# kezakool/flair-for-aigle

Measured on AMD Instinct MI355X. Metric: 512x512x5 tiles/sec (train fwd+bwd+AdamW), U-Net ResNet-34, 19 classes, higher is better.
Workload: dtype bf16; 1 GPU; synthetic 512x512x5 tiles, 19-class U-Net (ResNet-34 encoder), batch 32 per GPU, train step (BASELINE.json configs[1]); global_batch=32, tile=512, parallelism=dp1

## Files before the change

flair-for-aigle_amd/csrc/norm_pool.hip:

```cpp
#include "ffa_common.h"

#define FFA_EW_THREADS 256
#define FFA_MAX_PARTIALS 1024
#ifndef FFA_EW_UNROLL
#define FFA_EW_UNROLL 4
#endif

static inline int ew_grid(long long items) {
  long long g = (items + FFA_EW_THREADS - 1) / FFA_EW_THREADS;
  if (g > 256 * 8) g = 256 * 8;
  if (g < 1) g = 1;
  return (int)g;
}

static inline int ew_grid_c(long long nvec, int C) {
  int a = C / 8, b = FFA_EW_THREADS;
  while (b) {
    const int r = a % b;
    a = b;
    b = r;
  }
  const int m = (C / 8) / a;
  const int g = ew_grid((nvec + FFA_EW_UNROLL - 1) / FFA_EW_UNROLL) / m * m;
  return g < m ? m : g;
// ... 867 lines not shown
    red[t][e] = a[e];
    red[t][8 + e] = b[e];
  }
  __syncthreads();
  const int PL = FFA_COOP_THREADS / CG;
  for (int idx = t; idx < 2 * C; idx += FFA_COOP_THREADS) {
    const int which = idx / C, c = idx % C;
    const int g = c / 8, e = (c % 8) + which * 8;
    float s = 0.f;
    for (int q = 0; q < PL; ++q) s += red[q * CG + g][e];
    ws[((long long)blockIdx.x * 2 + which) * C + c] = s;
  }
  const unsigned nb = gridDim.x;
  bool ok = ffa_grid_barrier(sync + 0, nb, sync + 3);
  float* tot = ws + (long long)FFA_MAX_PARTIALS * 2 * C;
  for (int v = blockIdx.x; v < 2 * C; v += nb) {
    double s = 0.0;
    for (unsigned p = t; p < nb; p += FFA_COOP_THREADS) s += (double)ws[(long long)p * 2 * C + v];
#pragma unroll
    for (int o = 32; o > 0; o >>= 1) s += __shfl_xor(s, o, 64);
    if ((t & 63) == 0) dred[t >> 6] = s;
    __syncthreads();
    if (t == 0) {
      double r = 0.0;
      for (int wv = 0; wv < FFA_COOP_THREADS / 64; ++wv) r += dred[wv];
      tot[v] = (float)r;
    }
    __syncthreads();
  }
  ok = ffa_grid_barrier(sync + 1, nb, sync + 3) && ok;
  float kg[8], kx[8], k0[8];
#pragma unroll
  for (int e = 0; e < 8; ++e) {
    const float s = __hip_atomic_load(tot + c0 + e, __ATOMIC_RELAXED, __HIP_MEMORY_SCOPE_AGENT);
    const float q = __hip_atomic_load(tot + C + c0 + e, __ATOMIC_RELAXED, __HIP_MEMORY_SCOPE_AGENT);
    kg[e] = (gamma ? gamma[c0 + e] : 1.f) * rs[e];
    kx[e] = -kg[e] * rs[e] * q * inv_count;
    k0[e] = -kg[e] * s * inv_count - kx[e] * mu[e];
    if (blockIdx.x == 0 && t < CG) {
      dbeta[c0 + e] = s;
      dgamma[c0 + e] = q;
    }
  }
#pragma unroll
  for (int k = 0; k < ITEMS; ++k) {
    const long long i = tid_g + (long long)k * nthreads;
    if (i < nvec) {
      float xv[8], gv[8], o[8];
      ffa_unpack8_bf16(xr[k], xv);
      ffa_unpack8_bf16(gr[k], gv);
#pragma unroll
      for (int e = 0; e < 8; ++e) o[e] = kg[e] * gv[e] + kx[e] * xv[e] + k0[e];
      ffa_store8<ffa_bf16>(dx + i * 8, o);
      if (dres) *reinterpret_cast<ffa_u32x4*>(dres + i * 8) = gr[k];
    }
  }
  __syncthreads();
  if (t == 0) {
    __threadfence();
    if (atomicAdd(sync + 2, 1u) == nb - 1) {
      sync[0] = 0u;
      sync[1] = 0u;
      sync[2] = 0u;
      __threadfence();
    }
  }
  (void)ok;
}

extern "C" int ffa_bn_bwd_fused(int dtype, const void* x, const void* dy, const void* y, const float* gamma,
                                const float* beta, const float* mean, const float* rstd, void* dx, void* dres,
                                float* dgamma, float* dbeta, long long npix, int C, int relu, void* workspace,
                                long long workspace_bytes, unsigned* sync, hipStream_t stream) {
  FFA_REQUIRE(x && dy && dx && mean && rstd && dgamma && dbeta && workspace && sync, "bn_bwd_fused: null pointer");
  FFA_REQUIRE(relu >= 0 && relu <= 2 && (relu != 1 || y), "bn_bwd_fused: bad relu mode");
  static int cus = 0;
  if (cus == 0) {
    int dev = 0;
    hipDeviceProp_t prop;
    if (hipGetDevice(&dev) != hipSuccess || hipGetDeviceProperties(&prop, dev) != hipSuccess) return FFA_ERR_UNSUPPORTED;
    cus = prop.multiProcessorCount;
  }
  const int CG = C / 8;
  if (dtype != FFA_BF16 || C % 8 != 0 || CG < 1 || FFA_COOP_THREADS % CG != 0 || cus < 8 || cus > FFA_MAX_PARTIALS) {
    ffa_set_error("bn_bwd_fused: unsupported dtype / channel count %d", C);
    return FFA_ERR_UNSUPPORTED;
  }
  if (workspace_bytes < ffa_bn_workspace_bytes(C)) {
    ffa_set_error("bn_bwd_fused: workspace too small");
    return FFA_ERR_WORKSPACE;
  }
  const long long nvec = npix * CG;
  const long long nthreads = (long long)cus * FFA_COOP_THREADS;
  const long long items = (nvec + nthreads - 1) / nthreads;
  if (items > 16) {
    ffa_set_error("bn_bwd_fused: %lld vectors per thread exceed the register budget", items);
    return FFA_ERR_UNSUPPORTED;
  }
  const float inv_count = (float)(1.0 / (double)npix);
#define FFA_COOP_LAUNCH(N_)                                                                                      \
  hipLaunchKernelGGL(bn_bwd_coop_kernel<N_>, dim3(cus), dim3(FFA_COOP_THREADS), 0, stream, (const ffa_bf16*)x,   \
                     (const ffa_bf16*)dy, (const ffa_bf16*)y, gamma, beta, mean, rstd, (ffa_bf16*)dx,            \
                     (ffa_bf16*)dres, dgamma, dbeta, (float*)workspace, sync, nvec, C, relu, inv_count)
  if (items <= 4) FFA_COOP_LAUNCH(4);
  else FFA_COOP_LAUNCH(16);
#undef FFA_COOP_LAUNCH
  return ffa_check_launch("bn_bwd_fused");
}

extern "C" int ffa_bn_bwd_partials(int dtype, const void* x, const void* dy, const float* partials, long long nparts,
                                   const float* gamma, const float* beta, const float* mean, const float* rstd,
                                   void* dx, float* dgamma, float* dbeta, long long npix, int C, void* workspace,
                                   long long workspace_bytes, hipStream_t stream) {
  FFA_REQUIRE(x && dy && partials && dx && mean && rstd && dgamma && dbeta && workspace, "bn_bwd_partials: null pointer");
  FFA_REQUIRE(C % 8 == 0 && C >= 8 && C <= 8 * FFA_EW_THREADS && nparts > 0, "bn_bwd_partials: bad arguments");
  if (workspace_bytes < ffa_bn_workspace_bytes(C)) {
    ffa_set_error("bn_bwd_partials: workspace too small");
    return FFA_ERR_WORKSPACE;
  }
  float* ws = static_cast<float*>(workspace);
  float* coef = ws + (long long)FFA_MAX_PARTIALS * 2 * C;
  const float* src = partials;
  int n = (int)nparts;
  if (nparts > FFA_MAX_PARTIALS) {
    const int R = 64;
    hipLaunchKernelGGL(partials_fold_kernel, dim3(ffa_cdiv(C, 8), R), dim3(FFA_FIN_THREADS), 0, stream, partials, nparts,
                       C, R, ws);
    src = ws;
    n = R;
  }
  const long long nvec = npix * (C / 8);
  const float inv_count = (float)(1.0 / (double)npix);
  hipLaunchKernelGGL(bn_bwd_finalize_kernel, dim3(ffa_cdiv(C, 8)), dim3(FFA_FIN_THREADS), 0, stream, src, n, C, gamma, beta,
                     mean, rstd, inv_count, dgamma, dbeta, coef, 1);
  if (dtype == FFA_BF16)
    hipLaunchKernelGGL(bn_bwd_apply_kernel<ffa_bf16>, dim3(ew_grid_c(nvec, C)), dim3(FFA_EW_THREADS), 0, stream,
                       (const ffa_bf16*)x, (const ffa_bf16*)dy, (const ffa_bf16*)nullptr, coef, (ffa_bf16*)dx,
                       (ffa_bf16*)nullptr, nvec, C, 2);
  else
    hipLaunchKernelGGL(bn_bwd_apply_kernel<float>, dim3(ew_grid_c(nvec, C)), dim3(FFA_EW_THREADS), 0, stream, (const float*)x,
                       (const float*)dy, (const float*)nullptr, coef, (float*)dx, (float*)nullptr, nvec, C, 2);
  return ffa_check_launch("bn_bwd_partials");
}


template <typename T>
__global__ void __launch_bounds__(FFA_EW_THREADS)
maxpool_fwd_kernel(const T* __restrict__ x, T* __restrict__ y, uint8_t* __restrict__ idx, int B, int H, int W, int C,
                   int Ho, int Wo) {
  const unsigned CG = C / 8;
  const int oy = blockIdx.x % Ho;
  const long long b = blockIdx.x / Ho;
  const long long row = (long long)blockIdx.x * Wo * CG;
  for (unsigned j = threadIdx.x; j < (unsigned)Wo * CG; j += FFA_EW_THREADS) {
    const int ox = (int)(j / CG), g = (int)(j % CG);
    const long long i = row + j;
    float best[8];
    int bi[8];
#pragma unroll
    for (int e = 0; e < 8; ++e) {
      best[e] = -INFINITY;
      bi[e] = 0;
    }
    bool first = true;
#pragma unroll
    for (int r = 0; r < 3; ++r) {
      const int iy = oy * 2 - 1 + r;
      if (iy < 0 || iy >= H) continue;
#pragma unroll
      for (int s = 0; s < 3; ++s) {
        const int ix = ox * 2 - 1 + s;
        if (ix < 0 || ix >= W) continue;
        float v[8];
        ffa_load8<T>(x + ((b * H + iy) * W + ix) * C + g * 8, v);
#pragma unroll
        for (int e = 0; e < 8; ++e) {
          if (first || v[e] > best[e] || v[e] != v[e]) {
            best[e] = v[e];
            bi[e] = r * 3 + s;
          }
        }
        first = false;
      }
    }
    ffa_store8<T>(y + i * 8, best);
    uint32_t lo = bi[0] | (bi[1] << 8) | (bi[2] << 16) | (bi[3] << 24);
    uint32_t hi = bi[4] | (bi[5] << 8) | (bi[6] << 16) | (bi[7] << 24);
    *reinterpret_cast<uint2*>(idx + i * 8) = make_uint2(lo, hi);
  }
}

template <typename T>
__global__ void __launch_bounds__(FFA_EW_THREADS)
maxpool_bwd_kernel(const T* __restrict__ dy, const uint8_t* __restrict__ idx, const T* __restrict__ add,
                   T* __restrict__ dx, int B, int H, int W, int C, int Ho, int Wo) {
  const unsigned CG = C / 8;
  const int iy = blockIdx.x % H;
  const long long b = blockIdx.x / H;
  const long long row = (long long)blockIdx.x * W * CG;
  for (unsigned j = threadIdx.x; j < (unsigned)W * CG; j += FFA_EW_THREADS) {
    const int ix = (int)(j / CG), g = (int)(j % CG);
    const long long i = row + j;
    const int ny = (iy & 1) ? 2 : 1, nx = (ix & 1) ? 2 : 1;
    const int oy_c[2] = {(iy & 1) ? (iy + 1) >> 1 : iy >> 1, (iy - 1) >> 1};
    const int r_c[2] = {(iy & 1) ? 0 : 1, 2};
    const int ox_c[2] = {(ix & 1) ? (ix + 1) >> 1 : ix >> 1, (ix - 1) >> 1};
    const int s_c[2] = {(ix & 1) ? 0 : 1, 2};
    float acc[8];
#pragma unroll
    for (int e = 0; e < 8; ++e) acc[e] = 0.f;
    Raw8<T> addr, gr[4];
    uint2 kk[4];
    bool ok[4];
    if (add) addr.load(add + i * 8);
#pragma unroll
    for (int c = 0; c < 4; ++c) {
      const int cy = c >> 1, cx = c & 1;
      ok[c] = cy < ny && cx < nx && oy_c[cy] >= 0 && oy_c[cy] < Ho && ox_c[cx] >= 0 && ox_c[cx] < Wo;
      const long long o = ok[c] ? (((b * Ho + oy_c[cy]) * Wo + ox_c[cx]) * CG + g) * 8 : 0;
      kk[c] = *reinterpret_cast<const uint2*>(idx + o);
      gr[c].load(dy + o);
    }
    if (add) addr.get(acc);
#pragma unroll
    for (int c = 0; c < 4; ++c) {
      if (!ok[c]) continue;
      const int tap = r_c[c >> 1] * 3 + s_c[c & 1];
      float gv[8];
      gr[c].get(gv);
#pragma unroll
      for (int e = 0; e < 8; ++e) {
        const uint32_t word = e < 4 ? kk[c].x : kk[c].y;
        const int wq = (word >> (8 * (e & 3))) & 0xff;
        if (wq == tap) acc[e] += gv[e];
      }
    }
    ffa_store8<T>(dx + i * 8, acc);
  }
}

extern "C" int ffa_maxpool3x3s2_fwd(int dtype, const void* x, void* y, uint8_t* idx, int B, int H, int W, int C,
                                    hipStream_t stream) {
  FFA_REQUIRE(x && y && idx && C % 8 == 0, "maxpool_fwd: bad arguments");
  const int Ho = (H + 2 - 3) / 2 + 1, Wo = (W + 2 - 3) / 2 + 1;
  FFA_REQUIRE(B > 0 && (long long)B * Ho < (1LL << 31), "maxpool_fwd: too many rows");
  const int rows = B * Ho;
  if (dtype == FFA_BF16)
    hipLaunchKernelGGL(maxpool_fwd_kernel<ffa_bf16>, dim3(rows), dim3(FFA_EW_THREADS), 0, stream,
                       (const ffa_bf16*)x, (ffa_bf16*)y, idx, B, H, W, C, Ho, Wo);
  else
    hipLaunchKernelGGL(maxpool_fwd_kernel<float>, dim3(rows), dim3(FFA_EW_THREADS), 0, stream,
                       (const float*)x, (float*)y, idx, B, H, W, C, Ho, Wo);
  return ffa_check_launch("maxpool_fwd");
}

extern "C" int ffa_maxpool3x3s2_bwd(int dtype, const void* dy, const uint8_t* idx, const void* add, void* dx, int B,
                                    int H, int W, int C, hipStream_t stream) {
  FFA_REQUIRE(dy && dx && idx && C % 8 == 0, "maxpool_bwd: bad arguments");
  const int Ho = (H + 2 - 3) / 2 + 1, Wo = (W + 2 - 3) / 2 + 1;
  FFA_REQUIRE(B > 0 && (long long)B * H < (1LL << 31), "maxpool_bwd: too many rows");
  const int rows = B * H;
  if (dtype == FFA_BF16)
    hipLaunchKernelGGL(maxpool_bwd_kernel<ffa_bf16>, dim3(rows), dim3(FFA_EW_THREADS), 0, stream,
                       (const ffa_bf16*)dy, idx, (const ffa_bf16*)add, (ffa_bf16*)dx, B, H, W, C, Ho, Wo);
  else
    hipLaunchKernelGGL(maxpool_bwd_kernel<float>, dim3(rows), dim3(FFA_EW_THREADS), 0, stream,
                       (const float*)dy, idx, (const float*)add, (float*)dx, B, H, W, C, Ho, Wo);
  return ffa_check_launch("maxpool_bwd");
}

extern "C" int ffa_channel_sums(int dtype, const void* x, long long npix, int C, float* sum_out, float* sumsq_out,
                                void* workspace, long long workspace_bytes, hipStream_t stream) {
  FFA_REQUIRE(x && sum_out && sumsq_out && workspace, "channel_sums: null pointer");
  FFA_REQUIRE(C % 8 == 0 && C >= 8 && C <= 8 * FFA_EW_THREADS, "channel_sums: unsupported channel count %d", C);
  if (workspace_bytes < ffa_bn_workspace_bytes(C)) {
    ffa_set_error("channel_sums: workspace too small");
    return FFA_ERR_WORKSPACE;
  }
  const int nb = reduce_blocks(npix, C);
  float* ws = static_cast<float*>(workspace);
  if (dtype == FFA_BF16)
    hipLaunchKernelGGL((channel_reduce_kernel<ffa_bf16, StatOp>), dim3(nb), dim3(FFA_EW_THREADS), 0, stream,
                       (const ffa_bf16*)x, (const ffa_bf16*)nullptr, (const ffa_bf16*)nullptr, nullptr, nullptr, nullptr, nullptr, ws,
                       npix, C, 0, (ffa_bf16*)nullptr);
  else
    hipLaunchKernelGGL((channel_reduce_kernel<float, StatOp>), dim3(nb), dim3(FFA_EW_THREADS), 0, stream,
                       (const float*)x, (const float*)nullptr, (const float*)nullptr, nullptr, nullptr, nullptr, nullptr, ws, npix,
                       C, 0, (float*)nullptr);
  hipLaunchKernelGGL(bn_bwd_finalize_kernel, dim3(ffa_cdiv(C, 8)), dim3(FFA_FIN_THREADS), 0, stream, ws, nb, C,
                     (const float*)nullptr, (const float*)nullptr, (const float*)nullptr, (const float*)nullptr, 0.f,
                     sumsq_out, sum_out, (float*)nullptr);
  return ffa_check_launch("channel_sums");
}
```

flair-for-aigle_amd/csrc/resample_loss.hip:

```cpp
#include "ffa_common.h"

#include <stdlib.h>

#define FFA_EW_THREADS 256

static inline int ew_grid(long long items) {
  long long g = (items + FFA_EW_THREADS - 1) / FFA_EW_THREADS;
  if (g > 256 * 8) g = 256 * 8;
  if (g < 1) g = 1;
  return (int)g;
}


template <typename T>
__global__ void up2_concat_fwd_kernel(const T* __restrict__ lo, const T* __restrict__ skip, T* __restrict__ out, int B,
                                      int Hl, int Wl, int C1, int C2) {
  const int H = Hl * 2, W = Wl * 2, C = C1 + C2;
  const int CG = C / 8, CG1 = C1 / 8;
  const long long total = (long long)B * H * W * CG;
  for (long long i = blockIdx.x * (long long)blockDim.x + threadIdx.x; i < total;
       i += (long long)gridDim.x * blockDim.x) {
    const int g = (int)(i % CG);
    long long p = i / CG;
    const int x = (int)(p % W);
// ... 183 lines not shown
  else
    hipLaunchKernelGGL(bilinear_fwd_kernel<float>, dim3(ew_grid(items)), dim3(FFA_EW_THREADS), 0, stream,
                       (const float*)x, (float*)y, B, Hi, Wi, Ho, Wo, C, sy, sx);
  return ffa_check_launch("bilinear_fwd");
}

extern "C" long long ffa_bilinear_bwd_workspace_bytes(int B, int Hi, int Wi, int C) {
  (void)B; (void)Hi; (void)Wi; (void)C;
  return 0;
}

extern "C" int ffa_bilinear_bwd(int dtype, const void* dy, void* dx, int B, int Hi, int Wi, int Ho, int Wo, int C,
                                void* workspace, long long workspace_bytes, hipStream_t stream) {
  (void)workspace; (void)workspace_bytes;
  FFA_REQUIRE(dy && dx && C % 8 == 0 && B > 0 && Hi > 0 && Wi > 0 && Ho > 0 && Wo > 0, "bilinear_bwd: bad arguments");
  const float sy = (float)Hi / (float)Ho, sx = (float)Wi / (float)Wo;
  const long long items = (long long)B * Hi * Wi * (C / 8);
  if (dtype == FFA_BF16)
    hipLaunchKernelGGL(bilinear_bwd_kernel<ffa_bf16>, dim3(ew_grid(items)), dim3(FFA_EW_THREADS), 0, stream,
                       (const ffa_bf16*)dy, (ffa_bf16*)dx, B, Hi, Wi, Ho, Wo, C, sy, sx);
  else
    hipLaunchKernelGGL(bilinear_bwd_kernel<float>, dim3(ew_grid(items)), dim3(FFA_EW_THREADS), 0, stream,
                       (const float*)dy, (float*)dx, B, Hi, Wi, Ho, Wo, C, sy, sx);
  return ffa_check_launch("bilinear_bwd");
}


#define FFA_CE_BLOCKS 1024

__global__ void ce_weight_sum_kernel(const uint8_t* __restrict__ tgt, const float* __restrict__ w, int K,
                                     long long npix, float* __restrict__ parts, int vec16) {
  __shared__ float red[FFA_EW_THREADS / 64];
  __shared__ float wl[256];
  for (int i = threadIdx.x; i < 256; i += blockDim.x) wl[i] = (i < K) ? w[i] : 0.f;
  __syncthreads();
  float s = 0.f;
  const long long gid = blockIdx.x * (long long)blockDim.x + threadIdx.x;
  const long long stride = (long long)gridDim.x * blockDim.x;
  long long done = 0;
  if (vec16) {
    const long long n16 = npix / 16;
    for (long long i = gid; i < n16; i += stride) {
      const uint4 v = reinterpret_cast<const uint4*>(tgt)[i];
      const uint32_t q[4] = {v.x, v.y, v.z, v.w};
#pragma unroll
      for (int j = 0; j < 4; ++j)
#pragma unroll
        for (int b = 0; b < 4; ++b) s += wl[(q[j] >> (8 * b)) & 0xff];
    }
    done = n16 * 16;
  }
  for (long long i = done + gid; i < npix; i += stride) s += wl[tgt[i]];
  s = ffa_wave_sum(s);
  if ((threadIdx.x & 63) == 0) red[threadIdx.x >> 6] = s;
  __syncthreads();
  if (threadIdx.x == 0) {
    float tot = 0.f;
    for (int k = 0; k < FFA_EW_THREADS / 64; ++k) tot += red[k];
    parts[blockIdx.x] = tot;
  }
}

__device__ __forceinline__ double ce_sum_partials(const float* __restrict__ parts, int n) {
  double s = 0.0;
  for (int i = threadIdx.x; i < n; i += 64) s += (double)parts[i];
#pragma unroll
  for (int o = 32; o > 0; o >>= 1) s += __shfl_xor(s, o, 64);
  return s;
}

__global__ void ce_finalize_sum_kernel(const float* __restrict__ parts, int n, float* __restrict__ out) {
  const double s = ce_sum_partials(parts, n);
  if (threadIdx.x == 0) out[0] = (float)s;
}

__global__ void ce_finalize_loss_kernel(const float* __restrict__ parts, int n, const float* __restrict__ wsum,
                                        float* __restrict__ loss) {
  const double s = ce_sum_partials(parts, n);
  if (threadIdx.x == 0) loss[0] = (float)(s / (double)wsum[0]);
}

template <typename T>
__global__ void __launch_bounds__(FFA_EW_THREADS)
softmax_ce_kernel(const T* __restrict__ logits, const uint8_t* __restrict__ tgt, const float* __restrict__ w,
                  const float* __restrict__ wsum, const float* __restrict__ grad_scale, T* __restrict__ dlogits,
                  uint8_t* __restrict__ pred, float* __restrict__ parts, long long npix, int K, int Cp) {
  __shared__ float red[FFA_EW_THREADS / 64];
  float lsum = 0.f;
  float gs = 0.f;
  if (dlogits) gs = grad_scale[0] / wsum[0];
  const int nv = Cp / 8;
  for (long long i = blockIdx.x * (long long)blockDim.x + threadIdx.x; i < npix;
       i += (long long)gridDim.x * blockDim.x) {
    float z[FFA_CE_MAXK];
#pragma unroll
    for (int v = 0; v < FFA_CE_MAXK / 8; ++v) {
      if (v < nv) {
        float tmp[8];
        ffa_load8<T>(logits + i * Cp + v * 8, tmp);
#pragma unroll
        for (int e = 0; e < 8; ++e) z[v * 8 + e] = tmp[e];
      }
    }
    float m = -INFINITY;
    int am = 0;
#pragma unroll
    for (int k = 0; k < FFA_CE_MAXK; ++k) {
      if (k < K && z[k] > m) {
        m = z[k];
        am = k;
      }
    }
    const int t = tgt[i];
    const float wt = (t < K) ? w[t] : 0.f;
    float se = 0.f, dt = 0.f;
#pragma unroll
    for (int k = 0; k < FFA_CE_MAXK; ++k) {
      if (k < K) {
        const float d = z[k] - m;
        if (k == t) dt = d;
        z[k] = __expf(d);
        se += z[k];
      }
    }
    const float inv = 1.f / se;
    if (wt != 0.f) lsum += wt * (__logf(se) - dt);
    if (pred) pred[i] = (uint8_t)am;
    if (dlogits) {
      const float c = wt * gs;
#pragma unroll
      for (int v = 0; v < FFA_CE_MAXK / 8; ++v) {
        if (v < nv) {
          float o[8];
#pragma unroll
          for (int e = 0; e < 8; ++e) {
            const int k = v * 8 + e;
            o[e] = (k < K) ? c * (z[k] * inv - (k == t ? 1.f : 0.f)) : 0.f;
          }
          ffa_store8<T>(dlogits + i * Cp + v * 8, o);
        }
      }
    }
  }
  lsum = ffa_wave_sum(lsum);
  if ((threadIdx.x & 63) == 0) red[threadIdx.x >> 6] = lsum;
  __syncthreads();
  if (threadIdx.x == 0) {
    float tot = 0.f;
    for (int k = 0; k < FFA_EW_THREADS / 64; ++k) tot += red[k];
    parts[blockIdx.x] = tot;
  }
}

template <typename T, bool SUMS>
__global__ void __launch_bounds__(FFA_EW_THREADS)
softmax_ce_tiled_kernel(const T* __restrict__ logits, const uint8_t* __restrict__ tgt, const float* __restrict__ w,
                        const float* __restrict__ wsum, const float* __restrict__ grad_scale, T* __restrict__ dlogits,
                        uint8_t* __restrict__ pred, float* __restrict__ parts, float* __restrict__ parts_b,
                        long long npix, int K, int Cp) {
  constexpr int EPP = 16 / (int)sizeof(T);
  constexpr int MAXP = FFA_CE_MAXK / EPP;
  __shared__ __align__(16) unsigned char tile[FFA_EW_THREADS * (MAXP + 1) * 16];
  __shared__ float red[FFA_EW_THREADS / 64];
  const int tid = threadIdx.x;
  const int np = Cp / EPP;
  const int slots = np | 1;
  float bsum[SUMS ? EPP : 1];
#pragma unroll
  for (int k = 0; k < (SUMS ? EPP : 1); ++k) bsum[k] = 0.f;
  float lsum = 0.f;
  float gs = 0.f;
  if (dlogits) gs = grad_scale[0] / wsum[0];
  const long long ntiles = (npix + FFA_EW_THREADS - 1) / FFA_EW_THREADS;
  int loff[MAXP];
#pragma unroll
  for (int k = 0; k < MAXP; ++k) {
    const int idx = tid + FFA_EW_THREADS * k;
    loff[k] = ((idx / np) * slots + idx % np) * 16;
  }
  uint4 pre[MAXP];
  auto gload = [&](long long ti) {
    const long long base = ti * FFA_EW_THREADS;
    const long long left = npix - base;
    const int npc = (int)(left < FFA_EW_THREADS ? left : FFA_EW_THREADS) * np;
    const uint4* src = reinterpret_cast<const uint4*>(logits + base * Cp);
#pragma unroll
    for (int k = 0; k < MAXP; ++k) {
      const int idx = tid + FFA_EW_THREADS * k;
      if (k < np) pre[k] = idx < npc ? src[idx] : make_uint4(0u, 0u, 0u, 0u);
    }
  };
  long long ti = blockIdx.x;
  if (ti < ntiles) gload(ti);
  for (; ti < ntiles; ti += gridDim.x) {
#pragma unroll
    for (int k = 0; k < MAXP; ++k)
      if (k < np) *reinterpret_cast<uint4*>(tile + loff[k]) = pre[k];
    __syncthreads();
    if (ti + gridDim.x < ntiles) gload(ti + gridDim.x);
    const long long i = ti * FFA_EW_THREADS + tid;
    if (i < npix) {
      unsigned char* mine = tile + tid * slots * 16;
      float z[FFA_CE_MAXK];
#pragma unroll
      for (int v = 0; v < MAXP; ++v) {
        if (v < np) {
          const uint4 u = *reinterpret_cast<const uint4*>(mine + v * 16);
          if constexpr (sizeof(T) == 2) {
            z[v * 8 + 0] = __uint_as_float(u.x << 16);
            z[v * 8 + 1] = __uint_as_float(u.x & 0xffff0000u);
            z[v * 8 + 2] = __uint_as_float(u.y << 16);
            z[v * 8 + 3] = __uint_as_float(u.y & 0xffff0000u);
            z[v * 8 + 4] = __uint_as_float(u.z << 16);
            z[v * 8 + 5] = __uint_as_float(u.z & 0xffff0000u);
            z[v * 8 + 6] = __uint_as_float(u.w << 16);
            z[v * 8 + 7] = __uint_as_float(u.w & 0xffff0000u);
          } else {
            z[v * 4 + 0] = __uint_as_float(u.x);
            z[v * 4 + 1] = __uint_as_float(u.y);
            z[v * 4 + 2] = __uint_as_float(u.z);
            z[v * 4 + 3] = __uint_as_float(u.w);
          }
        }
      }
      float m = -INFINITY;
      int am = 0;
#pragma unroll
      for (int k = 0; k < FFA_CE_MAXK; ++k) {
        if (k < K && z[k] > m) {
          m = z[k];
          am = k;
        }
      }
      const int t = tgt[i];
      const float wt = (t < K) ? w[t] : 0.f;
      float se = 0.f, dt = 0.f;
#pragma unroll
      for (int k = 0; k < FFA_CE_MAXK; ++k) {
        if (k < K) {
          const float d = z[k] - m;
          if (k == t) dt = d;
          z[k] = __expf(d);
          se += z[k];
        }
      }
      const float inv = 1.f / se;
      if (wt != 0.f) lsum += wt * (__logf(se) - dt);
      if (pred) pred[i] = (uint8_t)am;
      if (dlogits) {
        const float c = wt * gs;
#pragma unroll
        for (int v = 0; v < MAXP; ++v) {
          if (v < np) {
            float o[EPP];
#pragma unroll
            for (int e = 0; e < EPP; ++e) {
              const int k = v * EPP + e;
              o[e] = (k < K) ? c * (z[k] * inv - (k == t ? 1.f : 0.f)) : 0.f;
            }
            uint4 u;
            if constexpr (sizeof(T) == 2) {
              u.x = ffa_pack_bf16x2(o[0], o[1]);
              u.y = ffa_pack_bf16x2(o[2], o[3]);
              u.z = ffa_pack_bf16x2(o[4], o[5]);
              u.w = ffa_pack_bf16x2(o[6], o[7]);
            } else {
              u = make_uint4(__float_as_uint(o[0]), __float_as_uint(o[1]), __float_as_uint(o[2]), __float_as_uint(o[3]));
            }
            *reinterpret_cast<uint4*>(mine + v * 16) = u;
          }
        }
      }
    }
    if (dlogits) {
      __syncthreads();
      const long long base = ti * FFA_EW_THREADS;
      const long long left = npix - base;
      const int npc = (int)(left < FFA_EW_THREADS ? left : FFA_EW_THREADS) * np;
      uint4* dst = reinterpret_cast<uint4*>(dlogits + base * Cp);
#pragma unroll
      for (int k = 0; k < MAXP; ++k) {
        const int idx = tid + FFA_EW_THREADS * k;
        if (k < np && idx < npc) {
          const uint4 u = *reinterpret_cast<const uint4*>(tile + loff[k]);
          dst[idx] = u;
          if constexpr (SUMS) {
            if constexpr (sizeof(T) == 2) {
              bsum[0] += __uint_as_float(u.x << 16);
              bsum[1] += __uint_as_float(u.x & 0xffff0000u);
              bsum[2] += __uint_as_float(u.y << 16);
              bsum[3] += __uint_as_float(u.y & 0xffff0000u);
              bsum[4] += __uint_as_float(u.z << 16);
              bsum[5] += __uint_as_float(u.z & 0xffff0000u);
              bsum[6] += __uint_as_float(u.w << 16);
              bsum[7] += __uint_as_float(u.w & 0xffff0000u);
            } else {
              bsum[0] += __uint_as_float(u.x);
              bsum[1] += __uint_as_float(u.y);
              bsum[2] += __uint_as_float(u.z);
              bsum[3] += __uint_as_float(u.w);
            }
          }
        }
      }
    }
    __syncthreads();
  }
  lsum = ffa_wave_sum(lsum);
  if ((threadIdx.x & 63) == 0) red[threadIdx.x >> 6] = lsum;
  if constexpr (SUMS) {
    float* wsums = reinterpret_cast<float*>(tile);
    if (threadIdx.x < (FFA_EW_THREADS / 64) * FFA_CE_MAXK) wsums[threadIdx.x] = 0.f;
    __syncthreads();
#pragma unroll
    for (int e = 0; e < EPP; ++e) {
      float t = bsum[e];
#pragma unroll
      for (int o = 32; o > 0; o >>= 1)
        if (o >= np) t += __shfl_xor(t, o, 64);
      if ((threadIdx.x & 63) < np) wsums[(threadIdx.x >> 6) * FFA_CE_MAXK + (threadIdx.x & 63) * EPP + e] = t;
    }
  }
  __syncthreads();
  if (threadIdx.x == 0) {
    float tot = 0.f;
    for (int k = 0; k < FFA_EW_THREADS / 64; ++k) tot += red[k];
    parts[blockIdx.x] = tot;
  }
  if constexpr (SUMS) {
    if (threadIdx.x < FFA_CE_MAXK) {
      const float* wsums = reinterpret_cast<const float*>(tile);
      float t = 0.f;
      for (int k = 0; k < FFA_EW_THREADS / 64; ++k) t += wsums[k * FFA_CE_MAXK + threadIdx.x];
      parts_b[(size_t)blockIdx.x * FFA_CE_MAXK + threadIdx.x] = t;
    }
  }
}

__global__ void __launch_bounds__(256) ce_finalize_cols_kernel(const float* __restrict__ parts_b, int nb, int Cp,
                                                               float* __restrict__ out) {
  __shared__ double sh[256];
  const int k = blockIdx.x;
  float v[FFA_CE_BLOCKS / 256];
#pragma unroll
  for (int j = 0; j < FFA_CE_BLOCKS / 256; ++j) {
    const int i = threadIdx.x + 256 * j;
    v[j] = i < nb ? parts_b[(size_t)i * FFA_CE_MAXK + k] : 0.f;
  }
  double s = 0.0;
#pragma unroll
  for (int j = 0; j < FFA_CE_BLOCKS / 256; ++j) s += (double)v[j];
  sh[threadIdx.x] = s;
  __syncthreads();
  if (threadIdx.x == 0) {
    double t = 0.0;
    for (int j = 0; j < 256; ++j) t += sh[j];
    out[k] = (float)t;
  }
}

extern "C" long long ffa_softmax_ce_workspace_bytes(void) {
  return (long long)(2 * FFA_CE_BLOCKS + 4 + FFA_CE_BLOCKS * FFA_CE_MAXK) * sizeof(float);
}

extern "C" int ffa_softmax_ce(int dtype, const void* logits, const uint8_t* targets, const float* class_weights,
                              const float* grad_scale, float* loss, float* wsum_out, void* dlogits, uint8_t* pred,
                              long long npix, int K, int Cp, void* workspace, long long workspace_bytes,
                              hipStream_t stream) {
  return ffa_softmax_ce_sums(dtype, logits, targets, class_weights, grad_scale, loss, wsum_out, dlogits, pred, nullptr,
                             npix, K, Cp, workspace, workspace_bytes, stream);
}

extern "C" int ffa_softmax_ce_sums(int dtype, const void* logits, const uint8_t* targets, const float* class_weights,
                                   const float* grad_scale, float* loss, float* wsum_out, void* dlogits, uint8_t* pred,
                                   float* dlogit_sums, long long npix, int K, int Cp, void* workspace,
                                   long long workspace_bytes, hipStream_t stream) {
  FFA_REQUIRE(logits && targets && class_weights && loss && wsum_out && workspace, "softmax_ce: null pointer");
  FFA_REQUIRE(K >= 1 && K <= FFA_CE_MAXK && Cp % 8 == 0 && Cp >= K && Cp <= FFA_CE_MAXK,
              "softmax_ce: unsupported class count %d (pitch %d)", K, Cp);
  FFA_REQUIRE(!dlogits || grad_scale, "softmax_ce: dlogits needs grad_scale");
  if (workspace_bytes < ffa_softmax_ce_workspace_bytes()) {
    ffa_set_error("softmax_ce: workspace too small");
    return FFA_ERR_WORKSPACE;
  }
  float* parts_w = static_cast<float*>(workspace);
  float* parts_l = parts_w + FFA_CE_BLOCKS;
  long long nb = (npix + FFA_EW_THREADS - 1) / FFA_EW_THREADS;
  if (nb > FFA_CE_BLOCKS) nb = FFA_CE_BLOCKS;
  if (nb < 1) nb = 1;
  hipLaunchKernelGGL(ce_weight_sum_kernel, dim3((int)nb), dim3(FFA_EW_THREADS), 0, stream, targets, class_weights, K,
                     npix, parts_w, (reinterpret_cast<uintptr_t>(targets) & 15) == 0 ? 1 : 0);
  hipLaunchKernelGGL(ce_finalize_sum_kernel, dim3(1), dim3(64), 0, stream, parts_w, (int)nb, wsum_out);
  const char* ct = getenv("FFA_CE_TILED");
  const bool tiled = !(ct && ct[0] == '0');
  const bool aligned = ((reinterpret_cast<uintptr_t>(logits) | reinterpret_cast<uintptr_t>(dlogits)) & 15) == 0;
  float* parts_b = parts_l + FFA_CE_BLOCKS + 4;
  const int pieces = Cp * (dtype == FFA_BF16 ? 2 : 4) / 16;
  if (dlogit_sums && !(tiled && aligned && dlogits && FFA_EW_THREADS % pieces == 0)) {
    ffa_set_error("softmax_ce_sums: needs dlogits, 16-byte aligned tensors, the tiled kernel and a pitch of 1, 2, 4 or 8 pieces");
    return FFA_ERR_UNSUPPORTED;
  }
  if (tiled && aligned && dlogit_sums) {
    if (dtype == FFA_BF16)
      hipLaunchKernelGGL((softmax_ce_tiled_kernel<ffa_bf16, true>), dim3((int)nb), dim3(FFA_EW_THREADS), 0, stream,
                         (const ffa_bf16*)logits, targets, class_weights, wsum_out, grad_scale, (ffa_bf16*)dlogits, pred,
                         parts_l, parts_b, npix, K, Cp);
    else
      hipLaunchKernelGGL((softmax_ce_tiled_kernel<float, true>), dim3((int)nb), dim3(FFA_EW_THREADS), 0, stream,
                         (const float*)logits, targets, class_weights, wsum_out, grad_scale, (float*)dlogits, pred,
                         parts_l, parts_b, npix, K, Cp);
    hipLaunchKernelGGL(ce_finalize_cols_kernel, dim3(Cp), dim3(256), 0, stream, parts_b, (int)nb, Cp, dlogit_sums);
  } else if (tiled && aligned) {
    if (dtype == FFA_BF16)
      hipLaunchKernelGGL((softmax_ce_tiled_kernel<ffa_bf16, false>), dim3((int)nb), dim3(FFA_EW_THREADS), 0, stream,
                         (const ffa_bf16*)logits, targets, class_weights, wsum_out, grad_scale, (ffa_bf16*)dlogits, pred,
                         parts_l, nullptr, npix, K, Cp);
    else
      hipLaunchKernelGGL((softmax_ce_tiled_kernel<float, false>), dim3((int)nb), dim3(FFA_EW_THREADS), 0, stream,
                         (const float*)logits, targets, class_weights, wsum_out, grad_scale, (float*)dlogits, pred,
                         parts_l, nullptr, npix, K, Cp);
  } else if (dtype == FFA_BF16)
    hipLaunchKernelGGL(softmax_ce_kernel<ffa_bf16>, dim3((int)nb), dim3(FFA_EW_THREADS), 0, stream,
                       (const ffa_bf16*)logits, targets, class_weights, wsum_out, grad_scale, (ffa_bf16*)dlogits, pred,
                       parts_l, npix, K, Cp);
  else
    hipLaunchKernelGGL(softmax_ce_kernel<float>, dim3((int)nb), dim3(FFA_EW_THREADS), 0, stream,
                       (const float*)logits, targets, class_weights, wsum_out, grad_scale, (float*)dlogits, pred,
                       parts_l, npix, K, Cp);
  hipLaunchKernelGGL(ce_finalize_loss_kernel, dim3(1), dim3(64), 0, stream, parts_l, (int)nb, wsum_out, loss);
  return ffa_check_launch("softmax_ce");
}

template <typename T>
__global__ void scale_inplace_kernel(T* __restrict__ x, long long nvec, const float* __restrict__ scale) {
  const float s = scale[0];
  if (s == 1.f) return;
  for (long long i = blockIdx.x * (long long)blockDim.x + threadIdx.x; i < nvec;
       i += (long long)gridDim.x * blockDim.x) {
    float v[8];
    ffa_load8<T>(x + i * 8, v);
#pragma unroll
    for (int e = 0; e < 8; ++e) v[e] *= s;
    ffa_store8<T>(x + i * 8, v);
  }
}

extern "C" int ffa_scale_inplace(int dtype, void* x, long long n, const float* scale, hipStream_t stream) {
  FFA_REQUIRE(x && scale && n % 8 == 0, "scale_inplace: bad arguments");
  const long long nvec = n / 8;
  if (dtype == FFA_BF16)
    hipLaunchKernelGGL(scale_inplace_kernel<ffa_bf16>, dim3(ew_grid(nvec)), dim3(FFA_EW_THREADS), 0, stream,
                       (ffa_bf16*)x, nvec, scale);
  else
    hipLaunchKernelGGL(scale_inplace_kernel<float>, dim3(ew_grid(nvec)), dim3(FFA_EW_THREADS), 0, stream, (float*)x,
                       nvec, scale);
  return ffa_check_launch("scale_inplace");
}


template <typename T>
__global__ void argmax_crop_kernel(const T* __restrict__ logits, uint8_t* __restrict__ out, int B, int H, int W, int K,
                                   int Cp, int y0, int x0, int h, int w) {
  const long long total = (long long)B * h * w;
  const int nv = Cp / 8;
  for (long long i = blockIdx.x * (long long)blockDim.x + threadIdx.x; i < total;
       i += (long long)gridDim.x * blockDim.x) {
    const int x = (int)(i % w);
    long long p = i / w;
    const int y = (int)(p % h);
    const long long b = p / h;
    const T* src = logits + ((b * H + y0 + y) * W + x0 + x) * Cp;
    float m = -INFINITY;
    int am = 0;
#pragma unroll
    for (int v = 0; v < FFA_CE_MAXK / 8; ++v) {
      if (v < nv) {
        float tmp[8];
        ffa_load8<T>(src + v * 8, tmp);
#pragma unroll
        for (int e = 0; e < 8; ++e) {
          const int k = v * 8 + e;
          if (k < K && tmp[e] > m) {
            m = tmp[e];
            am = k;
          }
        }
      }
    }
    out[i] = (uint8_t)am;
  }
}

template <typename T>
__global__ void class_prob_crop_kernel(const T* __restrict__ logits, uint8_t* __restrict__ out, int B, int H, int W,
                                       int K, int Cp, int y0, int x0, int h, int w) {
  const long long total = (long long)B * h * w;
  const int nv = Cp / 8;
  for (long long i = blockIdx.x * (long long)blockDim.x + threadIdx.x; i < total;
       i += (long long)gridDim.x * blockDim.x) {
    const int x = (int)(i % w);
    long long p = i / w;
    const int y = (int)(p % h);
    const long long b = p / h;
    const T* src = logits + ((b * H + y0 + y) * W + x0 + x) * Cp;
    float z[FFA_CE_MAXK];
#pragma unroll
    for (int v = 0; v < FFA_CE_MAXK / 8; ++v) {
      if (v < nv) {
        float tmp[8];
        ffa_load8<T>(src + v * 8, tmp);
#pragma unroll
        for (int e = 0; e < 8; ++e) z[v * 8 + e] = tmp[e];
      }
    }
    float m = -INFINITY;
#pragma unroll
    for (int k = 0; k < FFA_CE_MAXK; ++k)
      if (k < K) m = fmaxf(m, z[k]);
    float se = 0.f;
#pragma unroll
    for (int k = 0; k < FFA_CE_MAXK; ++k)
      if (k < K) {
        z[k] = expf(z[k] - m);
        se += z[k];
      }
#pragma unroll
    for (int k = 0; k < FFA_CE_MAXK; ++k)
      if (k < K) out[((b * K + k) * h + y) * (long long)w + x] = (uint8_t)rintf(z[k] / se * 255.f);
  }
}

template <typename T>
__global__ void label_conf_crop_kernel(const T* __restrict__ logits, uint8_t* __restrict__ out, int B, int H, int W,
                                       int K, int Cp, int y0, int x0, int h, int w) {
  const long long total = (long long)B * h * w;
  const long long plane = (long long)h * w;
  const int nv = Cp / 8;
  for (long long i = blockIdx.x * (long long)blockDim.x + threadIdx.x; i < total;
       i += (long long)gridDim.x * blockDim.x) {
    const int x = (int)(i % w);
    long long p = i / w;
    const int y = (int)(p % h);
    const long long b = p / h;
    const T* src = logits + ((b * H + y0 + y) * W + x0 + x) * Cp;
    float z[FFA_CE_MAXK];
#pragma unroll
    for (int v = 0; v < FFA_CE_MAXK / 8; ++v) {
      if (v < nv) {
        float tmp[8];
        ffa_load8<T>(src + v * 8, tmp);
#pragma unroll
        for (int e = 0; e < 8; ++e) z[v * 8 + e] = tmp[e];
      }
    }
    float m = -INFINITY, mm = -INFINITY;
    int am = 0;
#pragma unroll
    for (int k = 0; k < FFA_CE_MAXK; ++k)
      if (k < K) {
        m = fmaxf(m, z[k]);
        if (z[k] > mm) {
          mm = z[k];
          am = k;
        }
      }
    float se = 0.f, top = 0.f;
#pragma unroll
    for (int k = 0; k < FFA_CE_MAXK; ++k)
      if (k < K) {
        const float e = expf(z[k] - m);
        se += e;
        top = fmaxf(top, e);
      }
// ... 102 lines not shown
```

Baseline: 2470 tiles/s.

## Reuse maxpool window loads across output pairs and specialize CE kernel on padded width

The maxpool forward now computes two adjacent outputs per thread from one shared 3x5 window of loads, and the backward pass handles a 2x2 block of input pixels per thread so each dy/idx load serves up to four outputs. This is meant to cut redundant global reads. The tiled softmax-CE kernel is templated on the number of 16-byte pieces that actually hold classes, which skips the padded pieces. It also double-buffers prefetches with two register sets, and handles the target logit and its gradient with a separate scalar path. These changes add register pressure and code complexity.

```diff
diff --git a/flair-for-aigle_amd/csrc/norm_pool.hip b/flair-for-aigle_amd/csrc/norm_pool.hip
--- a/flair-for-aigle_amd/csrc/norm_pool.hip
+++ b/flair-for-aigle_amd/csrc/norm_pool.hip
@@ -1043,41 +1043,62 @@
   const int oy = blockIdx.x % Ho;
   const long long b = blockIdx.x / Ho;
   const long long row = (long long)blockIdx.x * Wo * CG;
-  for (unsigned j = threadIdx.x; j < (unsigned)Wo * CG; j += FFA_EW_THREADS) {
-    const int ox = (int)(j / CG), g = (int)(j % CG);
-    const long long i = row + j;
-    float best[8];
-    int bi[8];
-#pragma unroll
-    for (int e = 0; e < 8; ++e) {
-      best[e] = -INFINITY;
-      bi[e] = 0;
-    }
-    bool first = true;
-#pragma unroll
-    for (int r = 0; r < 3; ++r) {
-      const int iy = oy * 2 - 1 + r;
-      if (iy < 0 || iy >= H) continue;
-#pragma unroll
-      for (int s = 0; s < 3; ++s) {
-        const int ix = ox * 2 - 1 + s;
-        if (ix < 0 || ix >= W) continue;
-        float v[8];
-        ffa_load8<T>(x + ((b * H + iy) * W + ix) * C + g * 8, v);
-#pragma unroll
-        for (int e = 0; e < 8; ++e) {
-          if (first || v[e] > best[e] || v[e] != v[e]) {
-            best[e] = v[e];
-            bi[e] = r * 3 + s;
+  bool rok[3];
+  long long rbase[3];
+#pragma unroll
+  for (int r = 0; r < 3; ++r) {
+    const int iy = oy * 2 - 1 + r;
+    rok[r] = iy >= 0 && iy < H;
+    rbase[r] = (b * H + (iy < 0 ? 0 : iy >= H ? H - 1 : iy)) * W;
+  }
+  const unsigned pairs = ((unsigned)Wo + 1) / 2;
+  for (unsigned j = threadIdx.x; j < pairs * CG; j += FFA_EW_THREADS) {
+    const int p = (int)(j / CG), g = (int)(j % CG);
+    bool cok[5];
+    Raw8<T> v[3][5];
+#pragma unroll
+    for (int c = 0; c < 5; ++c) {
+      const int ix = p * 4 - 1 + c;
+      cok[c] = ix >= 0 && ix < W;
+      const int ixc = ix < 0 ? 0 : ix >= W ? W - 1 : ix;
+#pragma unroll
+      for (int r = 0; r < 3; ++r) v[r][c].load(x + ((rbase[r] + ixc) * C + g * 8));
+    }
+#pragma unroll
+    for (int o = 0; o < 2; ++o) {
+      const int ox = p * 2 + o;
+      if (ox >= Wo) continue;
+      float best[8];
+      int bi[8];
+#pragma unroll
+      for (int e = 0; e < 8; ++e) {
+        best[e] = -INFINITY;
+        bi[e] = 0;
+      }
+      bool first = true;
+#pragma unroll
+      for (int r = 0; r < 3; ++r) {
+#pragma unroll
+        for (int s = 0; s < 3; ++s) {
+          if (!rok[r] || !cok[2 * o + s]) continue;
+          float f[8];
+          v[r][2 * o + s].get(f);
+#pragma unroll
+          for (int e = 0; e < 8; ++e) {
+            if (first || f[e] > best[e] || f[e] != f[e]) {
+              best[e] = f[e];
+              bi[e] = r * 3 + s;
+            }
           }
+          first = false;
         }
-        first = false;
-      }
-    }
-    ffa_store8<T>(y + i * 8, best);
-    uint32_t lo = bi[0] | (bi[1] << 8) | (bi[2] << 16) | (bi[3] << 24);
-    uint32_t hi = bi[4] | (bi[5] << 8) | (bi[6] << 16) | (bi[7] << 24);
-    *reinterpret_cast<uint2*>(idx + i * 8) = make_uint2(lo, hi);
+      }
+      const long long i = row + (long long)ox * CG + g;
+      ffa_store8<T>(y + i * 8, best);
+      uint32_t lo = bi[0] | (bi[1] << 8) | (bi[2] << 16) | (bi[3] << 24);
+      uint32_t hi = bi[4] | (bi[5] << 8) | (bi[6] << 16) | (bi[7] << 24);
+      *reinterpret_cast<uint2*>(idx + i * 8) = make_uint2(lo, hi);
+    }
   }
 }
 
@@ -1086,47 +1107,63 @@
 maxpool_bwd_kernel(const T* __restrict__ dy, const uint8_t* __restrict__ idx, const T* __restrict__ add,
                    T* __restrict__ dx, int B, int H, int W, int C, int Ho, int Wo) {
   const unsigned CG = C / 8;
-  const int iy = blockIdx.x % H;
-  const long long b = blockIdx.x / H;
-  const long long row = (long long)blockIdx.x * W * CG;
-  for (unsigned j = threadIdx.x; j < (unsigned)W * CG; j += FFA_EW_THREADS) {
-    const int ix = (int)(j / CG), g = (int)(j % CG);
-    const long long i = row + j;
-    const int ny = (iy & 1) ? 2 : 1, nx = (ix & 1) ? 2 : 1;
-    const int oy_c[2] = {(iy & 1) ? (iy + 1) >> 1 : iy >> 1, (iy - 1) >> 1};
-    const int r_c[2] = {(iy & 1) ? 0 : 1, 2};
-    const int ox_c[2] = {(ix & 1) ? (ix + 1) >> 1 : ix >> 1, (ix - 1) >> 1};
-    const int s_c[2] = {(ix & 1) ? 0 : 1, 2};
-    float acc[8];
-#pragma unroll
-    for (int e = 0; e < 8; ++e) acc[e] = 0.f;
-    Raw8<T> addr, gr[4];
-    uint2 kk[4];
-    bool ok[4];
-    if (add) addr.load(add + i * 8);
-#pragma unroll
-    for (int c = 0; c < 4; ++c) {
-      const int cy = c >> 1, cx = c & 1;
-      ok[c] = cy < ny && cx < nx && oy_c[cy] >= 0 && oy_c[cy] < Ho && ox_c[cx] >= 0 && ox_c[cx] < Wo;
-      const long long o = ok[c] ? (((b * Ho + oy_c[cy]) * Wo + ox_c[cx]) * CG + g) * 8 : 0;
-      kk[c] = *reinterpret_cast<const uint2*>(idx + o);
-      gr[c].load(dy + o);
-    }
-    if (add) addr.get(acc);
-#pragma unroll
-    for (int c = 0; c < 4; ++c) {
-      if (!ok[c]) continue;
-      const int tap = r_c[c >> 1] * 3 + s_c[c & 1];
-      float gv[8];
-      gr[c].get(gv);
-#pragma unroll
-      for (int e = 0; e < 8; ++e) {
-        const uint32_t word = e < 4 ? kk[c].x : kk[c].y;
-        const int wq = (word >> (8 * (e & 3))) & 0xff;
-        if (wq == tap) acc[e] += gv[e];
-      }
-    }
-    ffa_store8<T>(dx + i * 8, acc);
+  const int HP = (H + 1) / 2;
+  const int a = blockIdx.x % HP;
+  const long long b = blockIdx.x / HP;
+  const bool oyok[2] = {true, a + 1 < Ho};
+  const bool iyok[2] = {true, 2 * a + 1 < H};
+  const unsigned pairs = ((unsigned)W + 1) / 2;
+  for (unsigned j = threadIdx.x; j < pairs * CG; j += FFA_EW_THREADS) {
+    const int bq = (int)(j / CG), g = (int)(j % CG);
+    const bool oxok[2] = {true, bq + 1 < Wo};
+    const bool ixok[2] = {true, 2 * bq + 1 < W};
+    Raw8<T> gr[2][2], addr[2][2];
+    uint2 kk[2][2];
+#pragma unroll
+    for (int cy = 0; cy < 2; ++cy)
+#pragma unroll
+      for (int cx = 0; cx < 2; ++cx) {
+        const long long o = (((b * Ho + (oyok[cy] ? a + cy : a)) * Wo + (oxok[cx] ? bq + cx : bq)) * CG + g) * 8;
+        kk[cy][cx] = *reinterpret_cast<const uint2*>(idx + o);
+        gr[cy][cx].load(dy + o);
+      }
+    long long ip[2][2];
+#pragma unroll
+    for (int py = 0; py < 2; ++py)
+#pragma unroll
+      for (int px = 0; px < 2; ++px) {
+        ip[py][px] = (((b * H + 2 * a + (iyok[py] ? py : 0)) * W + 2 * bq + (ixok[px] ? px : 0)) * CG + g) * 8;
+        if (add) addr[py][px].load(add + ip[py][px]);
+      }
+#pragma unroll
+    for (int py = 0; py < 2; ++py)
+#pragma unroll
+      for (int px = 0; px < 2; ++px) {
+        if (!iyok[py] || !ixok[px]) continue;
+        float acc[8];
+#pragma unroll
+        for (int e = 0; e < 8; ++e) acc[e] = 0.f;
+        if (add) addr[py][px].get(acc);
+#pragma unroll
+        for (int c = 0; c < 4; ++c) {
+          const int ny = py ? 2 : 1, nx = px ? 2 : 1;
+          const int qy = c >> 1, qx = c & 1;
+          if (qy >= ny || qx >= nx) continue;
+          const int cy = py ? 1 - qy : 0, cx = px ? 1 - qx : 0;
+          const int r = py ? 2 * qy : 1, s = px ? 2 * qx : 1;
+          if (!oyok[cy] || !oxok[cx]) continue;
+          const int tap = r * 3 + s;
+          float gv[8];
+          gr[cy][cx].get(gv);
+#pragma unroll
+          for (int e = 0; e < 8; ++e) {
+            const uint32_t word = e < 4 ? kk[cy][cx].x : kk[cy][cx].y;
+            const int wq = (word >> (8 * (e & 3))) & 0xff;
+            if (wq == tap) acc[e] += gv[e];
+          }
+        }
+        ffa_store8<T>(dx + ip[py][px], acc);
+      }
   }
 }
 
@@ -1150,7 +1187,7 @@
   FFA_REQUIRE(dy && dx && idx && C % 8 == 0, "maxpool_bwd: bad arguments");
   const int Ho = (H + 2 - 3) / 2 + 1, Wo = (W + 2 - 3) / 2 + 1;
   FFA_REQUIRE(B > 0 && (long long)B * H < (1LL << 31), "maxpool_bwd: too many rows");
-  const int rows = B * H;
+  const int rows = B * ((H + 1) / 2);
   if (dtype == FFA_BF16)
     hipLaunchKernelGGL(maxpool_bwd_kernel<ffa_bf16>, dim3(rows), dim3(FFA_EW_THREADS), 0, stream,
                        (const ffa_bf16*)dy, idx, (const ffa_bf16*)add, (ffa_bf16*)dx, B, H, W, C, Ho, Wo);
diff --git a/flair-for-aigle_amd/csrc/resample_loss.hip b/flair-for-aigle_amd/csrc/resample_loss.hip
--- a/flair-for-aigle_amd/csrc/resample_loss.hip
+++ b/flair-for-aigle_amd/csrc/resample_loss.hip
@@ -359,7 +359,7 @@
   }
 }
 
-template <typename T, bool SUMS>
+template <typename T, bool SUMS, int NPR>
 __global__ void __launch_bounds__(FFA_EW_THREADS)
 softmax_ce_tiled_kernel(const T* __restrict__ logits, const uint8_t* __restrict__ tgt, const float* __restrict__ w,
                         const float* __restrict__ wsum, const float* __restrict__ grad_scale, T* __restrict__ dlogits,
@@ -379,74 +379,84 @@
   float gs = 0.f;
   if (dlogits) gs = grad_scale[0] / wsum[0];
   const long long ntiles = (npix + FFA_EW_THREADS - 1) / FFA_EW_THREADS;
+  constexpr int NZ = NPR * EPP;
   int loff[MAXP];
 #pragma unroll
   for (int k = 0; k < MAXP; ++k) {
     const int idx = tid + FFA_EW_THREADS * k;
-    loff[k] = ((idx / np) * slots + idx % np) * 16;
-  }
-  uint4 pre[MAXP];
-  auto gload = [&](long long ti) {
+    loff[k] = idx % np < NPR ? ((idx / np) * slots + idx % np) * 16 : -1;
+  }
+  int goff[NPR], foff[NPR];
+#pragma unroll
+  for (int k = 0; k < NPR; ++k) {
+    const int j = tid + FFA_EW_THREADS * k;
+    goff[k] = (j / NPR) * np + j % NPR;
+    foff[k] = ((j / NPR) * slots + j % NPR) * 16;
+  }
+  uint4 pre0[NPR], pre1[NPR];
+  int tg0 = 0, tg1 = 0;
+  auto gload = [&](long long ti, uint4 (&pre)[NPR], int& tg) {
     const long long base = ti * FFA_EW_THREADS;
     const long long left = npix - base;
-    const int npc = (int)(left < FFA_EW_THREADS ? left : FFA_EW_THREADS) * np;
+    const int npx = (int)(left < FFA_EW_THREADS ? left : FFA_EW_THREADS);
     const uint4* src = reinterpret_cast<const uint4*>(logits + base * Cp);
 #pragma unroll
-    for (int k = 0; k < MAXP; ++k) {
-      const int idx = tid + FFA_EW_THREADS * k;
-      if (k < np) pre[k] = idx < npc ? src[idx] : make_uint4(0u, 0u, 0u, 0u);
-    }
+    for (int k = 0; k < NPR; ++k)
+      pre[k] = tid + FFA_EW_THREADS * k < npx * NPR ? src[goff[k]] : make_uint4(0u, 0u, 0u, 0u);
+    tg = tid < npx ? (int)tgt[base + tid] : 0;
   };
-  long long ti = blockIdx.x;
-  if (ti < ntiles) gload(ti);
-  for (; ti < ntiles; ti += gridDim.x) {
-#pragma unroll
-    for (int k = 0; k < MAXP; ++k)
-      if (k < np) *reinterpret_cast<uint4*>(tile + loff[k]) = pre[k];
+  auto do_tile = [&](long long ti, uint4 (&pre)[NPR], int& tg) {
+#pragma unroll
+    for (int k = 0; k < NPR; ++k) *reinterpret_cast<uint4*>(tile + foff[k]) = pre[k];
+    const int t = tg;
     __syncthreads();
-    if (ti + gridDim.x < ntiles) gload(ti + gridDim.x);
+    if (ti + 2 * (long long)gridDim.x < ntiles) gload(ti + 2 * (long long)gridDim.x, pre, tg);
     const long long i = ti * FFA_EW_THREADS + tid;
     if (i < npix) {
       unsigned char* mine = tile + tid * slots * 16;
-      float z[FFA_CE_MAXK];
-#pragma unroll
-      for (int v = 0; v < MAXP; ++v) {
-        if (v < np) {
-          const uint4 u = *reinterpret_cast<const uint4*>(mine + v * 16);
-          if constexpr (sizeof(T) == 2) {
-            z[v * 8 + 0] = __uint_as_float(u.x << 16);
-            z[v * 8 + 1] = __uint_as_float(u.x & 0xffff0000u);
-            z[v * 8 + 2] = __uint_as_float(u.y << 16);
-            z[v * 8 + 3] = __uint_as_float(u.y & 0xffff0000u);
-            z[v * 8 + 4] = __uint_as_float(u.z << 16);
-            z[v * 8 + 5] = __uint_as_float(u.z & 0xffff0000u);
-            z[v * 8 + 6] = __uint_as_float(u.w << 16);
-            z[v * 8 + 7] = __uint_as_float(u.w & 0xffff0000u);
-          } else {
-            z[v * 4 + 0] = __uint_as_float(u.x);
-            z[v * 4 + 1] = __uint_as_float(u.y);
-            z[v * 4 + 2] = __uint_as_float(u.z);
-            z[v * 4 + 3] = __uint_as_float(u.w);
-          }
-        }
+      float z[NZ];
+#pragma unroll
+      for (int v = 0; v < NPR; ++v) {
+        const uint4 u = *reinterpret_cast<const uint4*>(mine + v * 16);
+        if constexpr (sizeof(T) == 2) {
+          z[v * 8 + 0] = __uint_as_float(u.x << 16);
+          z[v * 8 + 1] = __uint_as_float(u.x & 0xffff0000u);
+          z[v * 8 + 2] = __uint_as_float(u.y << 16);
+          z[v * 8 + 3] = __uint_as_float(u.y & 0xffff0000u);
+          z[v * 8 + 4] = __uint_as_float(u.z << 16);
+          z[v * 8 + 5] = __uint_as_float(u.z & 0xffff0000u);
+          z[v * 8 + 6] = __uint_as_float(u.w << 16);
+          z[v * 8 + 7] = __uint_as_float(u.w & 0xffff0000u);
+        } else {
+          z[v * 4 + 0] = __uint_as_float(u.x);
+          z[v * 4 + 1] = __uint_as_float(u.y);
+          z[v * 4 + 2] = __uint_as_float(u.z);
+          z[v * 4 + 3] = __uint_as_float(u.w);
+        }
+      }
+      float zt = 0.f;
+      if (t < K) {
+        if constexpr (sizeof(T) == 2)
+          zt = __uint_as_float((uint32_t)*reinterpret_cast<const uint16_t*>(mine + t * 2) << 16);
+        else
+          zt = *reinterpret_cast<const float*>(mine + t * 4);
       }
       float m = -INFINITY;
       int am = 0;
 #pragma unroll
-      for (int k = 0; k < FFA_CE_MAXK; ++k) {
-        if (k < K && z[k] > m) {
+      for (int k = 0; k < NZ; ++k) {
+        if ((k < NZ - EPP || k < K) && z[k] > m) {
           m = z[k];
           am = k;
         }
       }
-      const int t = tgt[i];
       const float wt = (t < K) ? w[t] : 0.f;
-      float se = 0.f, dt = 0.f;
-#pragma unroll
-      for (int k = 0; k < FFA_CE_MAXK; ++k) {
-        if (k < K) {
+      float se = 0.f;
+      const float dt = t < K ? zt - m : 0.f;
+#pragma unroll
+      for (int k = 0; k < NZ; ++k) {
+        if (k < NZ - EPP || k < K) {
           const float d = z[k] - m;
-          if (k == t) dt = d;
           z[k] = __expf(d);
           se += z[k];
         }
@@ -457,25 +467,30 @@
       if (dlogits) {
         const float c = wt * gs;
 #pragma unroll
-        for (int v = 0; v < MAXP; ++v) {
-          if (v < np) {
-            float o[EPP];
-#pragma unroll
-            for (int e = 0; e < EPP; ++e) {
-              const int k = v * EPP + e;
-              o[e] = (k < K) ? c * (z[k] * inv - (k == t ? 1.f : 0.f)) : 0.f;
-            }
-            uint4 u;
-            if constexpr (sizeof(T) == 2) {
-              u.x = ffa_pack_bf16x2(o[0], o[1]);
-              u.y = ffa_pack_bf16x2(o[2], o[3]);
-              u.z = ffa_pack_bf16x2(o[4], o[5]);
-              u.w = ffa_pack_bf16x2(o[6], o[7]);
-            } else {
-              u = make_uint4(__float_as_uint(o[0]), __float_as_uint(o[1]), __float_as_uint(o[2]), __float_as_uint(o[3]));
-            }
-            *reinterpret_cast<uint4*>(mine + v * 16) = u;
+        for (int v = 0; v < NPR; ++v) {
+          float o[EPP];
+#pragma unroll
+          for (int e = 0; e < EPP; ++e) {
+            const int k = v * EPP + e;
+            o[e] = (k < NZ - EPP || k < K) ? c * (z[k] * inv) : 0.f;
           }
+          uint4 u;
+          if constexpr (sizeof(T) == 2) {
+            u.x = ffa_pack_bf16x2(o[0], o[1]);
+            u.y = ffa_pack_bf16x2(o[2], o[3]);
+            u.z = ffa_pack_bf16x2(o[4], o[5]);
+            u.w = ffa_pack_bf16x2(o[6], o[7]);
+          } else {
+            u = make_uint4(__float_as_uint(o[0]), __float_as_uint(o[1]), __float_as_uint(o[2]), __float_as_uint(o[3]));
+          }
+          *reinterpret_cast<uint4*>(mine + v * 16) = u;
+        }
+        if (t < K) {
+          const float gt = c * __builtin_fmaf(__expf(dt), inv, -1.f);
+          if constexpr (sizeof(T) == 2)
+            *reinterpret_cast<uint16_t*>(mine + t * 2) = (uint16_t)ffa_f32_to_bf16_bits(gt);
+          else
+            *reinterpret_cast<float*>(mine + t * 4) = gt;
         }
       }
     }
@@ -489,7 +504,7 @@
       for (int k = 0; k < MAXP; ++k) {
         const int idx = tid + FFA_EW_THREADS * k;
         if (k < np && idx < npc) {
-          const uint4 u = *reinterpret_cast<const uint4*>(tile + loff[k]);
+          const uint4 u = loff[k] >= 0 ? *reinterpret_cast<const uint4*>(tile + loff[k]) : make_uint4(0u, 0u, 0u, 0u);
           dst[idx] = u;
           if constexpr (SUMS) {
             if constexpr (sizeof(T) == 2) {
@@ -512,6 +527,16 @@
       }
     }
     __syncthreads();
+  };
+  long long ti = blockIdx.x;
+  if (ti < ntiles) gload(ti, pre0, tg0);
+  if (ti + gridDim.x < ntiles) gload(ti + gridDim.x, pre1, tg1);
+  while (ti < ntiles) {
+    do_tile(ti, pre0, tg0);
+    ti += gridDim.x;
+    if (ti >= ntiles) break;
+    do_tile(ti, pre1, tg1);
+    ti += gridDim.x;
   }
   lsum = ffa_wave_sum(lsum);
   if ((threadIdx.x & 63) == 0) red[threadIdx.x >> 6] = lsum;
@@ -564,6 +589,34 @@
     for (int j = 0; j < 256; ++j) t += sh[j];
     out[k] = (float)t;
   }
+}
+
+template <typename T, int NPR>
+static void ce_tiled_launch_n(int nb, hipStream_t stream, const T* logits, const uint8_t* tgt, const float* w,
+                              const float* wsum, const float* grad_scale, T* dlogits, uint8_t* pred, float* parts,
+                              float* parts_b, long long npix, int K, int Cp) {
+  if (parts_b)
+    hipLaunchKernelGGL((softmax_ce_tiled_kernel<T, true, NPR>), dim3(nb), dim3(FFA_EW_THREADS), 0, stream, logits, tgt, w,
+                       wsum, grad_scale, dlogits, pred, parts, parts_b, npix, K, Cp);
+  else
+    hipLaunchKernelGGL((softmax_ce_tiled_kernel<T, false, NPR>), dim3(nb), dim3(FFA_EW_THREADS), 0, stream, logits, tgt, w,
+                       wsum, grad_scale, dlogits, pred, parts, parts_b, npix, K, Cp);
+}
+
+template <typename T, typename... A>
+static void ce_tiled_launch(int nb, hipStream_t stream, const T* logits, const uint8_t* tgt, const float* w,
+                            const float* wsum, const float* grad_scale, T* dlogits, uint8_t* pred, float* parts,
+                            float* parts_b, long long npix, int K, int Cp) {
+  constexpr int EPP = 16 / (int)sizeof(T);
+#define FFA_CE_CASE(N)                                                                                                \
+  case N:                                                                                                             \
+    if constexpr (N <= FFA_CE_MAXK / EPP)                                                                             \
+      ce_tiled_launch_n<T, N>(nb, stream, logits, tgt, w, wsum, grad_scale, dlogits, pred, parts, parts_b, npix, K, Cp); \
+    break;
+  switch ((K + EPP - 1) / EPP) {
+    FFA_CE_CASE(1) FFA_CE_CASE(2) FFA_CE_CASE(3) FFA_CE_CASE(4) FFA_CE_CASE(5) FFA_CE_CASE(6) FFA_CE_CASE(7) FFA_CE_CASE(8)
+  }
+#undef FFA_CE_CASE
 }
 
 extern "C" long long ffa_softmax_ce_workspace_bytes(void) {
@@ -607,25 +660,15 @@
     ffa_set_error("softmax_ce_sums: needs dlogits, 16-byte aligned tensors, the tiled kernel and a pitch of 1, 2, 4 or 8 pieces");
     return FFA_ERR_UNSUPPORTED;
   }
-  if (tiled && aligned && dlogit_sums) {
+  if (tiled && aligned) {
     if (dtype == FFA_BF16)
-      hipLaunchKernelGGL((softmax_ce_tiled_kernel<ffa_bf16, true>), dim3((int)nb), dim3(FFA_EW_THREADS), 0, stream,
-                         (const ffa_bf16*)logits, targets, class_weights, wsum_out, grad_scale, (ffa_bf16*)dlogits, pred,
-                         parts_l, parts_b, npix, K, Cp);
+      ce_tiled_launch<ffa_bf16>((int)nb, stream, (const ffa_bf16*)logits, targets, class_weights, wsum_out, grad_scale,
+                                (ffa_bf16*)dlogits, pred, parts_l, dlogit_sums ? parts_b : nullptr, npix, K, Cp);
     else
-      hipLaunchKernelGGL((softmax_ce_tiled_kernel<float, true>), dim3((int)nb), dim3(FFA_EW_THREADS), 0, stream,
-                         (const float*)logits, targets, class_weights, wsum_out, grad_scale, (float*)dlogits, pred,
-                         parts_l, parts_b, npix, K, Cp);
-    hipLaunchKernelGGL(ce_finalize_cols_kernel, dim3(Cp), dim3(256), 0, stream, parts_b, (int)nb, Cp, dlogit_sums);
-  } else if (tiled && aligned) {
-    if (dtype == FFA_BF16)
-      hipLaunchKernelGGL((softmax_ce_tiled_kernel<ffa_bf16, false>), dim3((int)nb), dim3(FFA_EW_THREADS), 0, stream,
-                         (const ffa_bf16*)logits, targets, class_weights, wsum_out, grad_scale, (ffa_bf16*)dlogits, pred,
-                         parts_l, nullptr, npix, K, Cp);
-    else
-      hipLaunchKernelGGL((softmax_ce_tiled_kernel<float, false>), dim3((int)nb), dim3(FFA_EW_THREADS), 0, stream,
-                         (const float*)logits, targets, class_weights, wsum_out, grad_scale, (float*)dlogits, pred,
-                         parts_l, nullptr, npix, K, Cp);
+      ce_tiled_launch<float>((int)nb, stream, (const float*)logits, targets, class_weights, wsum_out, grad_scale,
+                             (float*)dlogits, pred, parts_l, dlogit_sums ? parts_b : nullptr, npix, K, Cp);
+    if (dlogit_sums)
+      hipLaunchKernelGGL(ce_finalize_cols_kernel, dim3(Cp), dim3(256), 0, stream, parts_b, (int)nb, Cp, dlogit_sums);
   } else if (dtype == FFA_BF16)
     hipLaunchKernelGGL(softmax_ce_kernel<ffa_bf16>, dim3((int)nb), dim3(FFA_EW_THREADS), 0, stream,
                        (const ffa_bf16*)logits, targets, class_weights, wsum_out, grad_scale, (ffa_bf16*)dlogits, pred,
```

Measured after the change: 2483 tiles/s (median of 6 runs). No clear change (+0.5%).
